# lmb-freiburg/understanding_flow_robustness

Hardware: AMD Instinct MI355X
Metric: attack-iters/s (higher is better)
Workload: dtype f32

## Files before the change

include/ufr_hip.h:

```cpp
#ifndef UFR_HIP_H_
#define UFR_HIP_H_

#include <stdint.h>

#ifdef __cplusplus
extern "C" {
#endif

#define UFR_ABI_VERSION 9

enum { UFR_F32 = 0, UFR_F64 = 1, UFR_F16 = 2 };
enum {
  UFR_OK = 0,
  UFR_EINVAL = -1,
  UFR_EUNSUPPORTED = -2,
  UFR_ELAUNCH = -3
};

typedef void* ufr_stream_t;

int ufr_abi_version(void);
const char* ufr_last_error(void);
int ufr_device_count(void);
const char* ufr_build_manifest(void);
// ... 337 lines not shown
                               void* c3a, long c3a_stride, void* c3b, long c3b_stride, float* c3_nchw, float* c3w_nchw,
                               const int* win, int B, int H, int W, int wh, int ww, int m2, int m3, ufr_stream_t stream);
int ufr_chunks_to_nchw(const void* planes, long plane_stride, const float* f32, int chunk0, const void* mask,
                       int mask_chunk0, float* out, int B, int C, int H, int W, float scale, float slope,
                       ufr_stream_t stream);
int ufr_nchw_cat_to_planes(const float* const* srcs, const int* channels, const int* dst_channel0, int nseg, void* planes,
                           long plane_stride, int chunk0, int chunks, int B, int H, int W, ufr_stream_t stream);
int ufr_chunks_to_nchw_cat(const float* g, int chunk0, int chunks, float* const* dsts, const int* channels, const int* src_channel0,
                           int nseg, const float* act0, float pos0, float neg0, int B, int H, int W, ufr_stream_t stream);
int ufr_grad_finalize(const float* g, int g_chunk0, const void* mask, int mask_chunk0, void* out, long out_plane_stride,
                      int out_chunk0, long M, int chunks, float slope, ufr_stream_t stream);

int ufr_conv1_direct(const float* frames_a, const float* frames_b, int Ba, int Bb, int H, int W, const double* mean,
                     const void* wimg, const float* bias, float slope, void* out_planes, long plane_stride, int out_chunk0,
                     ufr_stream_t stream);
int ufr_conv1_pack_planes(const float* frames_a, const float* frames_b, void* planes, long plane_stride, int Ba, int Bb, int H,
                          int W, const double* mean, ufr_stream_t stream);
int ufr_conv1_unpack_grad(const float* G, float* grad_frames, int N, int H, int W, ufr_stream_t stream);
int ufr_unshuffle_pack_planes(const float* x, void* planes, long plane_stride, int N, int C, int H, int W, ufr_stream_t stream);
int ufr_unshuffle_unpack_grad(const float* G, float* grad_x, int N, int C, int H, int W, ufr_stream_t stream);
int ufr_nchw_grad_to_planes(const float* grad, const float* act, void* planes, long plane_stride, int chunk0, int B, int C, int H,
                            int W, float slope, ufr_stream_t stream);
int ufr_window_gather_chunks(const float* src, float* dst, const int* win, int n_win, int N, int N_dst, int chunks, int Hs, int Ws,
                             int wh, int ww, int level_stride, int margin, ufr_stream_t stream);

int ufr_normalize_frames(const float* frames_a, const float* frames_b, float* out, int Ba, int Bb, int C, int H, int W,
                         const double* mean, ufr_stream_t stream);

int ufr_corr_forward_planes_window(const void* f1_planes, const void* f2_planes, long in_plane_stride, void* out_planes,
                                   long out_plane_stride, int out_chunk0, int B, int C, int H, int W, int patch,
                                   int dilation_patch, float scale, float slope, const int* win, int level_stride,
                                   int win_cells, ufr_stream_t stream);

int ufr_corr_backward_window_fused(const float* f1, const float* f2, const float* G, int g_chunk0, float g_scale,
                                   const float* G_redir, float* grad_window, int B, int C, int H, int W, int patch,
                                   int dilation_patch, const int* win, int level_stride, int wh, int ww, int margin,
                                   ufr_stream_t stream);

int ufr_corr_forward_planes(const void* f1_planes, const void* f2_planes, long in_plane_stride, void* out_planes,
                            long out_plane_stride, int out_chunk0, int B, int C, int H, int W, int patch,
                            int dilation_patch, float scale, float slope, ufr_stream_t stream);
int ufr_flow_head_planes_forward(const void* planes, long plane_stride, int chunk0, int chunks, const float* wpk, int w_chunks,
                                 const float* bias, float* out, int B, int H, int W, ufr_stream_t stream);
int ufr_flow_head_planes_forward_mfma(const void* planes, long plane_stride, int chunk0, int chunks, const void* wmf, int w_chunks,
                                      const float* bias, float* out, int B, int H, int W, ufr_stream_t stream);
int ufr_deconv_flow_tail_backward_mfma(const void* grad_planes, long plane_stride, int chunk0, int chunks, const void* wmf,
                                       int w_chunks, float* G, int g_chunks, int out_chunk, int B, int H, int W, ufr_stream_t stream);
int ufr_flow_head_planes_backward(const float* grad_y, const float* wpk, int w_chunks, float* G, int g_chunks, int chunk0, int chunks,
                                  int B, int H, int W, int accumulate, ufr_stream_t stream);
int ufr_flow_head_planes_backward_finalize(const float* grad_y, const float* wpk, int w_chunks, float* G, int g_chunks, int chunk0,
                                           int chunks, int B, int H, int W, int accumulate, const void* mask_planes, void* out_planes,
                                           long out_plane_stride, int fin_chunk0, int fin_chunks, float slope, ufr_stream_t stream);
#define UFR_PF_REGION_BAND 1
#define UFR_PF_REGION_WINDOW 2
int ufr_flow_head_planes_backward_regions(const float* grad_y, const float* wpk, int w_chunks, float* G, int g_chunks, int chunk0,
                                          int chunks, int B, int H, int W, int accumulate, int head_chunks, int region,
                                          const int* origin, int origin_stride, int origin_div, int reg_h, int reg_w, int margin,
                                          float* head_out, int head_out_images, const void* mask_planes, void* out_planes,
                                          long out_plane_stride, int fin_chunk0, int fin_chunks, float slope, ufr_stream_t stream);
int ufr_upfeat_planes_forward_mfma(const void* planes, long plane_stride, int chunk0, int chunks, const void* wmf, int w_chunks,
                                   const float* bias, float* out, int B, int H, int W, ufr_stream_t stream);
int ufr_upfeat_planes_backward(const float* grad_y, const float* wpk, int w_chunks, float* G, int g_chunks, int chunk0, int chunks,
                               int B, int H, int W, int accumulate, ufr_stream_t stream);
int ufr_flow_up_planes_forward(const float* x, const float* w, const float* bias, void* planes, long plane_stride,
                               int chunk, int B, int H, int W, ufr_stream_t stream);
int ufr_flow_up_planes_backward(const float* G, int chunk, const float* w, float* grad_x, int B, int H, int W,
// ... 38 lines not shown
```

understanding_flow_robustness_amd/_lib.py:

```python
from __future__ import annotations

import ctypes as C
import os

import torch

_HERE = os.path.dirname(os.path.abspath(__file__))
LIB_PATH = os.environ.get("UFR_HIP_LIB") or os.path.join(_HERE, "lib", "libufr_hip.so")
UFR_F32, UFR_F64, UFR_F16 = 0, 1, 2
ABI_VERSION = 9
_lib = None


class CorrParams(C.Structure):
    _fields_ = [(n, C.c_int) for n in (
        "kH", "kW", "patchH", "patchW", "padH", "padW", "dilationH", "dilationW",
        "dilation_patchH", "dilation_patchW", "dH", "dW")]


UFR_MAX_LEVELS = 8


class Pyramid(C.Structure):
    _fields_ = [("num_levels", C.c_int),
# ... 176 lines not shown
    "ufr_flow_head_planes_forward_mfma": [_vp, _l, _i, _i, _vp, _i, _vp, _vp, _i, _i, _i, _vp],
    "ufr_deconv_flow_tail_backward_mfma": [_vp, _l, _i, _i, _vp, _i, _vp, _i, _i, _i, _i, _i, _vp],
    "ufr_flow_head_planes_backward": [_vp, _vp, _i, _vp, _i, _i, _i, _i, _i, _i, _i, _vp],
    "ufr_flow_head_planes_backward_finalize": [_vp, _vp, _i, _vp, _i, _i, _i, _i, _i, _i, _i, _vp, _vp, _l, _i, _i, _f, _vp],
    "ufr_flow_head_planes_backward_regions": [_vp, _vp, _i, _vp, _i, _i, _i, _i, _i, _i, _i, _i, _i, _vp, _i, _i, _i, _i, _i, _vp, _i,
                                              _vp, _vp, _l, _i, _i, _f, _vp],
    "ufr_unshuffle_pack_planes": [_vp, _vp, _l, _i, _i, _i, _i, _vp],
    "ufr_unshuffle_unpack_grad": [_vp, _vp, _i, _i, _i, _i, _vp],
    "ufr_conv3x3s2_c3_planes": [_vp, _vp, _vp, _f, _vp, _l, _i, _i, _i, _i, _i, _vp],
    "ufr_conv3x3_c16_planes": [_vp, _l, _i, _vp, _vp, _f, _vp, _l, _i, _i, _i, _i, _vp],
    "ufr_cm_norm_stats": [_vp, _vp, _vp, _l, _i, _i, _f, _vp],
    "ufr_cm_norm_apply": [_vp, _vp, _vp, _l, _i, _vp, _l, _i, _l, _i, _i, _i, _i, _vp],
    "ufr_cm_norm_stats_apply": [_vp, _vp, _vp, _f, _vp, _l, _i, _vp, _l, _i, _l, _i, _i, _i, _i, _vp],
    "ufr_cm_norm_backward": [_vp, _vp, _vp, _i, _vp, _vp, _vp, _vp, _l, _i, _l, _i, _i, _i, _vp],
    "ufr_cm_masked_copy": [_vp, _vp, _l, _vp, _l, _vp],
    "ufr_raft_flow_patches": [_vp, _vp, _l, _i, _i, _i, _i, _vp],
    "ufr_raft_motion_finish_slabs": [_vp, _i, _i, _i, _vp, _f, _vp, _l, _vp, _l, _i, _vp, _i, _i, _i, _vp],
    "ufr_raft_motion_finish": [_vp, _l, _vp, _l, _i, _vp, _i, _i, _i, _vp],
    "ufr_raft_coords_step": [_vp, _vp, _vp, _vp, _vp, _l, _vp],
    "ufr_grad_finalize_consume": [_vp, _vp, _vp, _l, _l, _i, _f, _vp],
    "ufr_gru_gates_cm_forward": [_vp, _vp, _l, _i, _vp, _l, _i, _l, _i, _vp],
    "ufr_gru_gates_cm_forward_slabs": [_vp, _i, _i, _vp, _vp, _vp, _vp, _l, _i, _vp, _l, _i, _l, _i, _vp],
    "ufr_gru_blend_cm_forward_slabs": [_vp, _i, _i, _vp, _vp, _vp, _vp, _vp, _l, _i, _vp, _l, _i, _l, _i, _vp],
    "ufr_gru_blend_cm_forward": [_vp, _vp, _vp, _l, _i, _vp, _l, _i, _l, _i, _vp],
    "ufr_gru_blend_cm_backward": [_vp, _vp, _vp, _l, _i, _vp, _vp, _l, _i, _vp, _vp, _l, _i, _vp, _vp],
    "ufr_gru_gates_cm_backward": [_vp, _vp, _l, _i, _vp, _vp, _vp, _l, _i, _vp, _l, _i, _i, _vp, _vp],
    "ufr_altcorr_pyramid_forward": [_vp, _vp, _vp, _vp, _i, _i, _i, _i, _i, _f, _vp],
    "ufr_altcorr_pyramid_backward": [_vp, _vp, _vp, _vp, _vp, _vp, _i, _i, _i, _i, _i, _f, _i, _vp],
    "ufr_altcorr_pyramid_backward_cm": [_vp, _vp, _vp, _vp, _vp, _vp, _i, _i, _i, _i, _i, _f, _i, _vp],
    "ufr_upfeat_planes_forward_mfma": [_vp, _l, _i, _i, _vp, _i, _vp, _vp, _i, _i, _i, _vp],
    "ufr_upfeat_planes_backward": [_vp, _vp, _i, _vp, _i, _i, _i, _i, _i, _i, _i, _vp],
    "ufr_flow_up_planes_forward": [_vp, _vp, _vp, _vp, _l, _i, _i, _i, _i, _vp],
    "ufr_flow_up_planes_backward": [_vp, _i, _vp, _vp, _i, _i, _i, _i, _vp],
    "ufr_corr_forward_planes_window": [_vp, _vp, _l, _vp, _l, _i, _i, _i, _i, _i, _i, _i, _f, _f, _vp, _i, _i, _vp],
    "ufr_corr_forward_planes": [_vp, _vp, _l, _vp, _l, _i, _i, _i, _i, _i, _i, _i, _f, _f, _vp],
    "ufr_convex_upsample_forward": [_vp, _vp, _vp, _i, _i, _i, _vp],
    "ufr_convex_upsample_backward": [_vp, _vp, _vp, _vp, _vp, _vp, _i, _i, _i, _vp],
    "ufr_affine_resample_f64": [_vp, _vp, _i, _i, _i, _i, _i, _d, _d, _d, _d, _d, _d, _i, _vp],
    "ufr_patch_place": [_vp, _vp, _vp, _i, _i, _i, _vp, _vp, _vp, _i, _i, _i, _i, _vp],
    "ufr_patch_crop_f64": [_vp, _vp, _vp, _i, _i, _i, _i, _i, _i, _i, _vp],
    "ufr_resample_u8_horizontal": [_vp, _vp, _i, _i, _i, _i, _i, _vp, _vp, _i, _vp],
    "ufr_resample_u8_vertical": [_vp, _vp, _i, _i, _i, _i, _vp, _vp, _i, _vp],
    "ufr_u8_to_tensor": [_vp, _vp, _i, _i, _i, _i, _i, _i, _i, _f, _vp],
    "ufr_kitti_flow_decode": [_vp, _vp, _i, _i, _vp],
    "ufr_host_png_unfilter": [_vp, _vp, _i, _i, _i],
    "ufr_igemm_clock_probe": [_vp, _i],
    "ufr_altcorr_planes_prepare": [_vp, _vp, _l, _l, _i, _vp],
    "ufr_altcorr_planes_forward": [_vp, _l, C.POINTER(AltCorrPlaneLevels), _vp, _vp, _i, _i, _i, _i, _i, _f, _vp],
    "ufr_conv1_direct": [_vp, _vp, _i, _i, _i, _i, _vp, _vp, _vp, _f, _vp, _l, _i, _vp],
    "ufr_train_loss": [C.POINTER(TrainLossDesc), _vp],
    "ufr_grad_norm": [C.POINTER(AdamwSeg), _i, _f, _vp, _l, _vp, _vp],
    "ufr_adamw_step": [C.POINTER(AdamwSeg), _i, C.POINTER(AdamwHyper), _vp, _vp],
    "ufr_sweep_paste": [_vp, _vp, _vp, _vp, _vp, _vp, _vp, _vp, _i, _i, _i, _i, _i, _f, _f, C.POINTER(ConeChain), _i, _i, _vp, _vp, _vp],
    "ufr_sweep_metrics": [_vp, _vp, _vp, _vp, _vp, _i, _i, _i, _i, _i, _i, _i, _i, _vp, _l, _vp, _i, _i, _vp],
}
PLAIN = {"ufr_abi_version": (C.c_int, []), "ufr_last_error": (C.c_char_p, []),
         "ufr_device_count": (C.c_int, []), "ufr_build_manifest": (C.c_char_p, []),
         "ufr_igemm_variant_fallbacks": (C.c_int, []),
         "ufr_conv3x3_c2_workspace_floats": (C.c_long, [_i, _i, _i, _i]),
         "ufr_cm_norm_workspace_doubles": (C.c_long, [_l, _i, _i]),
         "ufr_resample2d_backward_workspace_bytes": (C.c_long, [_i, _i, _i]),
         "ufr_pwc_warp_backward_workspace_bytes": (C.c_long, [_i, _i, _i]),
         "ufr_altcorr_pyramid_workspace_bytes": (C.c_long, [_i, _i, _i, _i, _i, _i]),
         "ufr_train_loss_workspace_doubles": (C.c_long, [_i, _i, C.POINTER(C.c_int), C.POINTER(C.c_int)]),
         "ufr_grad_norm_partials": (C.c_long, [C.POINTER(AdamwSeg), _i]),
         "ufr_sweep_metrics_workspace_doubles": (C.c_long, [_i])}
# ... 263 lines not shown
```

understanding_flow_robustness_amd/csrc/correlation_planes.hip:

```cpp
#include "ufr_common.h"

namespace {

typedef __attribute__((ext_vector_type(8))) __bf16 bf16x8;
typedef __attribute__((ext_vector_type(4))) float f32x4;

__device__ constexpr int PROD_A[6] = {2, 0, 1, 1, 0, 0};
__device__ constexpr int PROD_B[6] = {0, 2, 1, 0, 1, 0};
__device__ __attribute__((aligned(64))) unsigned corr_zero_page[16];

__device__ __forceinline__ void glds16(const __bf16* src, __bf16* lds_wave_base) {
  __builtin_amdgcn_global_load_lds(src, lds_wave_base, 16, 0, 0);
}

__device__ __forceinline__ void split3(float v, __bf16& a, __bf16& b, __bf16& c) {
  a = (__bf16)v;
  const float r1 = v - (float)a;
  b = (__bf16)r1;
  c = (__bf16)(r1 - (float)b);
}

constexpr int P = 21, R = 10, KCH = 8;
constexpr int OT = 24;

// ... 136 lines not shown
        if (two) asm volatile("s_waitcnt vmcnt(6)" ::: "memory"); else asm volatile("s_waitcnt vmcnt(3)" ::: "memory");
      } else {
        asm volatile("s_waitcnt vmcnt(0)" ::: "memory");
      }
      asm volatile("s_waitcnt lgkmcnt(0)" ::: "memory");
      __builtin_amdgcn_s_barrier();
      cur = cur == 2 ? 0 : cur + 1;
      if (sl == KH - 1 && kh == 0) {
#pragma unroll
        for (int tt = 0; tt < 3; ++tt) {
          const f32x4 o = *reinterpret_cast<const f32x4*>(part + 4 * tt);
          acc[tt][0] += o[0]; acc[tt][1] += o[1]; acc[tt][2] += o[2]; acc[tt][3] += o[3];
        }
        write_row(dy, acc, false);
      }
    }
    t = tn;
  }
}

template <int NW>
int launch_corr_planes(const __bf16* a, const __bf16* b, long in_plane_stride, __bf16* o, long out_plane_stride, int out_chunk0,
                       int B, int H, int W, int ni, float scale, float slope, hipStream_t st, const int* win = nullptr,
                       int win_div = 1) {
  {
    hipError_t e = ufr::ensure_dynamic_lds(reinterpret_cast<const void*>(corr_fwd_planes_k2_kernel<NW>), corr_planes_k2_lds_bytes<NW>());
    if (e != hipSuccess) return ufr::fail(UFR_ELAUNCH, "correlation (planes): %s", hipGetErrorString(e));
  }
  corr_fwd_planes_k2_kernel<NW><<<dim3(win ? 1 : ufr::ceil_div(ni, 16 * NW), 2, B * H), 128 * NW, corr_planes_k2_lds_bytes<NW>(), st>>>(
      a, b, in_plane_stride, o, out_plane_stride, out_chunk0, B, H, W, scale, slope, win, win_div);
  return UFR_OK;
}

}

extern "C" int ufr_corr_forward_planes(const void* f1_planes, const void* f2_planes, long in_plane_stride, void* out_planes,
                                       long out_plane_stride, int out_chunk0, int B, int C, int H, int W, int patch,
                                       int dilation_patch, float scale, float slope, ufr_stream_t stream) {
  UFR_REQUIRE(f1_planes && f2_planes && out_planes, "correlation (planes): null pointer");
  UFR_REQUIRE(B > 0 && H > 0 && W > 0 && (long)B * H < 65536 && out_chunk0 >= 0, "correlation (planes): bad shape");
  if (C != 32 * KCH || patch != P || dilation_patch != 2)
    return ufr::fail(UFR_EUNSUPPORTED, "correlation (planes): built for FlowNetC's configuration (256 channels, patch 21, "
                                       "dilation_patch 2); got C=%d patch=%d dilation_patch=%d", C, patch, dilation_patch);
  const int ni = (W + 1) / 2;
  hipStream_t st = ufr::as_stream(stream);
  const __bf16* a = static_cast<const __bf16*>(f1_planes);
  const __bf16* b = static_cast<const __bf16*>(f2_planes);
  __bf16* o = static_cast<__bf16*>(out_planes);
  const int waves = ufr::ceil_div(ni, 16);
  int rc;
  if (waves <= 2) rc = launch_corr_planes<2>(a, b, in_plane_stride, o, out_plane_stride, out_chunk0, B, H, W, ni, scale, slope, st);
  else if (waves <= 4 || waves > 5 * 2)
    rc = launch_corr_planes<4>(a, b, in_plane_stride, o, out_plane_stride, out_chunk0, B, H, W, ni, scale, slope, st);
  else
    rc = launch_corr_planes<5>(a, b, in_plane_stride, o, out_plane_stride, out_chunk0, B, H, W, ni, scale, slope, st);
  if (rc != UFR_OK) return rc;
  return ufr::launched("corr_fwd_planes_kernel");
}

extern "C" int ufr_corr_forward_planes_window(const void* f1_planes, const void* f2_planes, long in_plane_stride, void* out_planes,
                                              long out_plane_stride, int out_chunk0, int B, int C, int H, int W, int patch,
                                              int dilation_patch, float scale, float slope, const int* win, int level_stride,
                                              int win_cells, ufr_stream_t stream) {
  UFR_REQUIRE(f1_planes && f2_planes && out_planes && win, "correlation (planes, window): null pointer");
  UFR_REQUIRE(B > 0 && H > 0 && W > 0 && (long)B * H < 65536 && out_chunk0 >= 0 && level_stride > 0 && win_cells > 0,
              "correlation (planes, window): bad shape");
  if (C != 32 * KCH || patch != P || dilation_patch != 2 || win_cells + 4 * R > 63)
    return ufr::fail(UFR_EUNSUPPORTED, "correlation (planes, window): 256 channels, patch 21, dilation_patch 2, windows of at most "
                                       "23 cells; got C=%d patch=%d dilation_patch=%d cells=%d", C, patch, dilation_patch, win_cells);
  int rc = launch_corr_planes<2>(static_cast<const __bf16*>(f1_planes), static_cast<const __bf16*>(f2_planes), in_plane_stride,
                                 static_cast<__bf16*>(out_planes), out_plane_stride, out_chunk0, B, H, W, (W + 1) / 2, scale, slope,
                                 ufr::as_stream(stream), win, level_stride);
  if (rc != UFR_OK) return rc;
  return ufr::launched("corr_fwd_planes_k2_kernel (window)");
}
```

understanding_flow_robustness_amd/flownetc_engine.py:

```python
from __future__ import annotations

import os

import torch
from ._lib import engine_cache as _engine_cache

from . import _lib as L
from . import igemm as ig

_HEADS = ((6, 1024), (5, 1026), (4, 770), (3, 386), (2, 194))


def _pack_flow_head(weight: torch.Tensor) -> torch.Tensor:
    cin = weight.shape[1]
    chunks = ig.pad32(cin) // 32
    w = torch.zeros(2, chunks * 32, 9, dtype=torch.float32, device=weight.device)
    w[:, :cin] = weight.detach().float().reshape(2, cin, 9)
    return w.view(2, chunks, 32, 9).permute(1, 3, 0, 2).contiguous()


def _pack_flow_head_mfma(weight: torch.Tensor) -> torch.Tensor:
    cin = weight.shape[1]
    chunks = ig.pad32(cin) // 32
    w = torch.zeros(chunks * 32, 32, dtype=torch.float32, device=weight.device)
# ... 13 lines not shown


class FlowNetCHeadEngine:
    def __init__(self, net, B: int, H: int, W: int, device):
        if H % 64 or W % 64:
            raise ValueError("FlowNetC head engine: frame sides must be multiples of 64")
        L.lib()
        self.net, self.B, self.H, self.W, self.dev = net, int(B), int(H), int(W), torch.device(device)
        g = {s: (H // s, W // s) for s in (4, 8, 16, 32, 64)}
        self.grid = g
        P = lambda s, chunks: ig.Planes(B, g[s][0], g[s][1], chunks, self.dev)
        G = lambda s, chunks: ig.GradSum(B, g[s][0], g[s][1], chunks, self.dev)
        self.siamese = hasattr(net, "conv_redir")
        self.c3a_p, self.c3b_p = (P(8, 8), P(8, 8)) if self.siamese else (None, None)
        self.in31, self.cat3, self.cat2 = P(8, 15 if self.siamese else 8), P(8, 13), P(4, 7)
        self.c4a, self.cat4 = P(16, 16), P(16, 25)
        self.c5a, self.cat5 = P(32, 16), P(32, 33)
        self.c6a, self.c6 = P(64, 32), P(64, 32)
        f32 = dict(dtype=torch.float32, device=self.dev)
        self.flow = {k: torch.zeros(B, 2, *g[2 ** k], **f32) for k in (6, 5, 4, 3, 2)}
        self.G_cat2, self.G_cat3, self.G_cat4, self.G_cat5 = G(4, 7), G(8, 13), G(16, 25), G(32, 33)
        self.G_c6, self.G_in31, self.G_c3a = G(64, 32), G(8, 15 if self.siamese else 8), G(8, 8)
        self.gz_cat2, self.gz_cat3, self.gz_cat4, self.gz_cat5 = P(4, 7), P(8, 13), P(16, 25), P(32, 33)
        self.gz_c6, self.gz_c6a, self.gz_c5a, self.gz_c4a = P(64, 32), P(64, 32), P(32, 16), P(16, 16)
        self.gz_in31 = P(8, 15) if self.siamese else None
        self.g_flow = {k: torch.zeros(B, 2, *g[2 ** k], **f32) for k in (6, 5, 4, 3)}
        self.g_corr = torch.zeros(B, 21, 21, *g[8], **f32)
        self.g_c2a = torch.zeros(B, 128, *g[4], **f32)
        self.g_c3a, self.g_c3a_redir, self.g_c3b = (torch.zeros(B, 256, *g[8], **f32) for _ in range(3))
        self.c3_nchw = torch.zeros(2 * B, 256, *g[8], **f32)
        self._prefix = None
        self.flow_out, self.flow_scale = self.flow[2], float(getattr(net, "div_flow", 20.0))
        self._wprefixes, self._wprefix = {}, None
        self._build_launches()

    def _conv(self, name):
        return getattr(self.net, name)[0]

    def _bias(self, conv):
        if conv.bias is None:
            return torch.zeros(conv.out_channels, dtype=torch.float32, device=self.dev)
        return conv.bias.detach().float().contiguous()

    def _stem_layers(self):
        from .plane_graph import stem_stages
        return [(name, block[0], lvl) for lvl, stage in enumerate(stem_stages(self.net), 1) for name, block in stage]

    def _build_launches(self):
        net, g, B = self.net, self.grid, self.B
        plans = []

        def plan(wi, x, in_chunk0, rows, out_hw, **kw):
            M = B * rows[0] * rows[1]
            pk = [len(t) * wi.KC for _, _, t in wi.phases]
            kw.setdefault("variant", self._variant_for(wi))
            bm, target = self._tile_rows_and_slots(wi, kw)
            S = ig.splitk_for(M, wi.Npad, max(pk), len(wi.phases), phase_ktiles=pk, bm=bm, target=target)
            kw["variant"], S = ig.tuned(wi, M, kw, kw["variant"], S, rows=rows)
            plans.append((wi, x, in_chunk0, rows, out_hw, S, kw))
            return len(plans) - 1

        self._pipe_variant = {"0": 2, "5": 5}.get(os.environ.get("UFR_IGEMM_PIPE", "6"), 6)

        fwd, bwd = {}, {}
        cw = lambda n, s, p: ig.conv_forward_weights(self._conv(n).weight, s, p)
        cb = lambda n, s, p: ig.conv_backward_weights(self._conv(n).weight, s, p)
# ... 133 lines not shown
        pk = P["packed"]
        L.check(L.lib().ufr_conv1_pack_planes(L.ptr(a), L.ptr(b.contiguous()) if b is not None else None, L.ptr(pk.t),
                                              pk.plane_stride, int(a.shape[0]), nb, int(a.shape[2]), int(a.shape[3]),
                                              L.ptr(mean), L.stream()), "conv1 pack")
        P["conv1"]()

    def prefix_full(self, frames_a: torch.Tensor, frames_b: torch.Tensor):
        if self._prefix is None:
            self._build_prefix()
        B = self.B

        def chain(h, frames, out):
            P = self._prefix[h]
            self._conv1(P, frames, None)
            for _, launch, _ in P["layers"]:
                launch()
            (self.c3a_p if h == "a" else self.c3b_p).to_nchw(256, 0, out=out)
        chain("a", frames_a, self.c3_nchw[:B])
        chain("b", frames_b, self.c3_nchw[B:])
        self._c3a, self._c3b = self.c3_nchw[:B], self.c3_nchw[B:]

    def load_prefix_features(self, c2_all: torch.Tensor, c3_all: torch.Tensor):
        B = self.B
        self.cat2.load_nchw(c2_all[:B].contiguous(), 0)
        self.c3_nchw.copy_(c3_all[:2 * B])
        self._c3a, self._c3b = self.c3_nchw[:B], self.c3_nchw[B:]
        self.c3a_p.load_nchw(self._c3a, 0)
        self.c3b_p.load_nchw(self._c3b, 0)

    def scatter_window_features(self, c2_w: torch.Tensor, c3_w: torch.Tensor, win: torch.Tensor, wh: int, ww: int, m2: int, m3: int):
        lib, B, st = L.lib(), self.B, L.stream()
        h4, w4 = self.grid[4]
        h8, w8 = self.grid[8]
        L.check(lib.ufr_window_scatter_planes(L.ptr(c2_w), L.ptr(self.cat2.t), self.cat2.plane_stride, 0, L.ptr(win), B, B, 128,
                                              h4, w4, wh // 4, ww // 4, 4, m2, st), "window -> planes (conv2)")
        for k, dst in ((0, self.c3a_p), (1, self.c3b_p)):
            L.check(lib.ufr_window_scatter_planes(L.ptr(c3_w[k * B:]), L.ptr(dst.t), dst.plane_stride, 0, L.ptr(win), B, B, 256,
                                                  h8, w8, wh // 8, ww // 8, 8, m3, st), "window -> planes (conv3)")
        L.check(lib.ufr_window_scatter(L.ptr(c3_w), L.ptr(self.c3_nchw), L.ptr(win), B, 2 * B, 256, h8, w8, wh // 8, ww // 8, 8,
                                       m3, st), "window -> nchw (conv3)")

    def _build_window_prefix(self, wh: int, ww: int):
        B2, dev = 2 * self.B, self.dev
        f32 = dict(dtype=torch.float32, device=dev)
        h2, w2, h4, w4, h8, w8 = wh // 2, ww // 2, wh // 4, ww // 4, wh // 8, ww // 8
        layers = self._stem_layers()
        n = len(layers)
        tap2 = max(i for i, (_, _, lvl) in enumerate(layers) if lvl == 2)
        acts = [ig.Planes(B2, wh >> lvl, ww >> lvl, ig.pad32(conv.out_channels) // 32, dev) for _, conv, lvl in layers]
        gz = [ig.Planes(B2, wh >> lvl, ww >> lvl, ig.pad32(conv.out_channels) // 32, dev) for _, conv, lvl in layers]
        G_p = ig.GradSum(B2, h2 + 3, w2 + 2, 1, dev)
        G_gw2 = ig.GradSum(B2, h4, w4, 4, dev)
        grid = lambda i: (wh >> layers[i][2], ww >> layers[i][2])
        plans, names = [], []
        for i in range(1, n):
            name, conv, _ = layers[i]
            plans.append((ig.conv_forward_weights(conv.weight, conv.stride[0], conv.padding[0]), acts[i - 1], grid(i), grid(i),
                          dict(out_planes=acts[i], bias=self._bias(conv), variant=4)))
            names.append(name)
        for i in range(n - 1, 0, -1):
            name, conv, _ = layers[i]
            kw = dict(add=G_gw2, mask=acts[i - 1], out_planes=gz[i - 1]) if i - 1 == tap2 else dict(out_planes=gz[i - 1], mask=acts[i - 1])
            plans.append((ig.conv_backward_weights(conv.weight, conv.stride[0], conv.padding[0]), gz[i], grid(i), grid(i - 1), kw))
            names.append(name + "_bwd")
        plans.append((ig.conv1_packed_backward_weights(layers[0][1].weight), gz[0], (h2 + 3, w2 + 2), (h2 + 3, w2 + 2),
                      dict(out_f32=G_p)))
# ... 8 lines not shown
        ws = torch.empty(need, **f32)
        launches = [ig.make_launch(wi, x, 0, rows, out_hw, splitk=S, ws=ws if S > 1 else None, **kw)
                    for (wi, x, rows, out_hw, kw), S in zip(plans, sized)]
        chain = [(name, launch, p[0]) for name, launch, p in zip(names, launches, plans)]
        P = dict(hw=(wh, ww), c1=acts[0], c2=acts[tap2], c3=acts[-1], gz_c3=gz[-1], gz_c2=gz[tap2], G_gw2=G_gw2, ws=ws,
                 acts=acts, gz=gz, fwd=chain[:n - 1], bwd=chain[n - 1:],
                 G_p=G_p, gxw=torch.zeros(B2, 3, wh, ww, **f32),
                 c2_nchw=torch.zeros(B2, 128, h4, w4, **f32), c3_nchw=torch.zeros(B2, 256, h8, w8, **f32))
        P.update({name: launch for name, launch, _ in chain})
        P.update({name + "_wi": wi for name, _, wi in chain})
        P.update(self._conv1_launch(B2, wh, ww, acts[0]))
        self._wprefixes[(wh, ww)] = P
        self._bound_wprefixes()
        return P

    MAX_WINDOW_PREFIXES = 4

    def _bound_wprefixes(self):
        while len(self._wprefixes) > self.MAX_WINDOW_PREFIXES:
            del self._wprefixes[next(iter(self._wprefixes))]

    def window_prefix(self, wh: int, ww: int) -> dict:
        P = self._wprefixes.pop((int(wh), int(ww)), None)
        if P is None:
            P = self._build_window_prefix(int(wh), int(ww))
        else:
            self._wprefixes[(int(wh), int(ww))] = P
        self._wprefix = P
        return P

    def window_prefix_forward(self, xw: torch.Tensor, win: torch.Tensor, m2: int, m3: int, c2_nchw: bool = True):
        wh, ww = int(xw.shape[2]), int(xw.shape[3])
        P = self.window_prefix(wh, ww)
        self._conv1(P, xw.detach(), None)
        for _, launch, _ in P["fwd"]:
            launch()
        c2, c3, H, W = P["c2"], P["c3"], self.H, self.W
        L.check(L.lib().ufr_window_features_planes(
            L.ptr(c2.t), c2.plane_stride, L.ptr(c3.t), c3.plane_stride, L.ptr(self.cat2.t), self.cat2.plane_stride,
            L.ptr(self.c3a_p.t), self.c3a_p.plane_stride, L.ptr(self.c3b_p.t), self.c3b_p.plane_stride, L.ptr(self.c3_nchw),
            L.ptr(P["c3_nchw"]), L.ptr(win), self.B, H, W, wh, ww, int(m2), int(m3), L.stream()), "window features -> planes")
        if c2_nchw:
            c2.to_nchw(128, 0, out=P["c2_nchw"])

    def window_gather_conv2_gradient(self, win: torch.Tensor, m2: int):
        P = self._wprefix
        wh, ww = P["hw"]
        h4, w4 = self.grid[4]
        L.check(L.lib().ufr_window_gather_chunks(L.ptr(self.G_cat2.t), L.ptr(P["G_gw2"].t), L.ptr(win), self.B, self.B, 2 * self.B, 4,
                                                 h4, w4, wh // 4, ww // 4, 4, int(m2), L.stream()), "window gather (chunks)")

    def window_prefix_backward(self, gw3: torch.Tensor, gw2: torch.Tensor | None = None, unpack: bool = True) -> torch.Tensor:
        P, B = self._wprefix, self.B
        wh, ww = P["hw"]
        if gw2 is not None:
            full = torch.zeros(2 * B, 128, wh // 4, ww // 4, dtype=torch.float32, device=self.dev)
            full[:B] = gw2
            P["G_gw2"].t.copy_(full.view(2 * B, 4, 32, wh // 4, ww // 4).permute(1, 0, 3, 4, 2).reshape(4, -1, 32))
        gz = P["gz_c3"]
        L.check(L.lib().ufr_nchw_grad_to_planes(L.ptr(gw3), L.ptr(P["c3_nchw"]), L.ptr(gz.t), gz.plane_stride, 0, 2 * B, 256, wh // 8,
                                                ww // 8, ig.LEAKY, L.stream()), "window gradient -> planes")
        for _, launch, _ in P["bwd"]:
            launch()
        if not unpack:
            return P["G_p"].t
        L.check(L.lib().ufr_conv1_unpack_grad(L.ptr(P["G_p"].t), L.ptr(P["gxw"]), 2 * B, wh, ww, L.stream()), "conv1 unpack")
# ... 175 lines not shown
                                                   L.ptr(dst.t), dst.plane_stride, chunk, self.B, f.shape[2], f.shape[3],
                                                   L.stream()), "upsampled_flow forward")

    def _deconv_tail(self, k):
        src, chunk0, chunks, Gd, out_chunk, (h, w) = self.tail_args[k]
        L.check(L.lib().ufr_deconv_flow_tail_backward_mfma(L.ptr(src.t), src.plane_stride, chunk0, chunks, L.ptr(self.tail_w[k]),
                                                           self.tail_w[k].shape[0], L.ptr(Gd.t), Gd.chunks, out_chunk, self.B, h, w, L.stream()),
                "deconv data gradient, flow channels")

    def _up_backward(self, k):
        G, chunk = self.up_G[k]
        f = self.g_flow[k]
        L.check(L.lib().ufr_flow_up_planes_backward(L.ptr(G.t), chunk, L.ptr(self.up_w[k]), L.ptr(f), self.B, f.shape[2],
                                                    f.shape[3], 0, L.stream()), "upsampled_flow backward")

    def _finalize(self, Gs, mask, out, chunk0, chunks):
        L.check(L.lib().ufr_grad_finalize(L.ptr(Gs.t), chunk0, L.ptr(mask.t), chunk0, L.ptr(out.t), out.plane_stride, chunk0,
                                          Gs.M, chunks, ig.LEAKY, L.stream()), "gradient finalize")

    def _forward_trunk(self, c2: torch.Tensor, c3: torch.Tensor) -> torch.Tensor:
        L.require_hip(c2, "c2")
        L.require_hip(c3, "c3")
        self.cat2.load_nchw(c2, 0)
        self.in31.load_nchw(c3, 0)
        for name in ("conv3_1", "conv4", "conv4_1", "conv5", "conv5_1", "conv6", "conv6_1"):
            self.fwd[name]()
        self._pf_forward(6)
        for k in (5, 4, 3, 2):
            self._up_forward(k + 1)
            self.fwd[f"deconv{k}"]()
            self._pf_forward(k)
        return self.flow[2]

    def forward_cached(self, band=None) -> torch.Tensor:
        return self.forward(None, self._c3a, self._c3b, band)

    def forward(self, c2a: torch.Tensor | None, c3a: torch.Tensor, c3b: torch.Tensor, band=None) -> torch.Tensor:
        if not self.siamese:
            return self._forward_trunk(c2a, c3a)
        for t, name in ((c3a, "c3a"), (c3b, "c3b")):
            L.require_hip(t, name)
        self._c3a, self._c3b = c3a, c3b
        inc = False
        if band is not None:
            self.attach_band(band)
            inc = bool(band.width and band.incremental and band.inc_layers)
        if c2a is not None:
            L.require_hip(c2a, "c2a")
            self.cat2.load_nchw(c2a, 0)
            self.c3a_p.load_nchw(c3a, 0)
            self.c3b_p.load_nchw(c3b, 0)
        if inc and band.cone_win is not None and band.cone_hw[1] // 8 <= 23:
            L.check(L.lib().ufr_corr_forward_planes_window(L.ptr(self.c3a_p.t), L.ptr(self.c3b_p.t), self.c3a_p.plane_stride,
                                                           L.ptr(self.in31.t), self.in31.plane_stride, 1, self.B, 256, *self.grid[8],
                                                           21, 2, 1.0 / 256.0, ig.LEAKY, L.ptr(band.cone_win), 8,
                                                           band.cone_hw[1] // 8, L.stream()), "correlation forward (planes, window)")
        else:
            L.check(L.lib().ufr_corr_forward_planes(L.ptr(self.c3a_p.t), L.ptr(self.c3b_p.t), self.c3a_p.plane_stride,
                                                    L.ptr(self.in31.t), self.in31.plane_stride, 1, self.B, 256, *self.grid[8], 21, 2,
                                                    1.0 / 256.0, ig.LEAKY, L.stream()), "correlation forward (planes)")
        for name in ("conv_redir", "conv3_1", "conv4", "conv4_1"):
            (self.fwd_band if inc else self.fwd)[name]()
        for name in ("conv5", "conv5_1", "conv6", "conv6_1"):
            self.fwd[name]()
        self._pf_forward(6)
        for k in (5, 4, 3, 2):
            self._up_forward(k + 1)
            self.fwd[f"deconv{k}"]()
            self._pf_forward(k)
        return self.flow[2]

    def backward(self, g_flow2: torch.Tensor, band=None, fused_window: bool = True, skip_unread: bool = True):
        L.require_hip(g_flow2, "g_flow2")
        B = self.B
        banded = band is not None and bool(band.width)
        if band is not None:
            self.attach_band(band)
        gz = {2: (self.G_cat2, self.cat2, self.gz_cat2, 4, 2), 3: (self.G_cat3, self.cat3, self.gz_cat3, 8, 4),
              4: (self.G_cat4, self.cat4, self.gz_cat4, 16, 8), 5: (self.G_cat5, self.cat5, self.gz_cat5, 16, 16)}
        fuse = os.environ.get("UFR_FUSE_FINALIZE", "1") != "0"
        fin = lambda k: (gz[k][1], gz[k][2], gz[k][3], gz[k][4]) if fuse else None
        eng_window = bool(fused_window and band is not None and getattr(band, "eng_window", False)
                          and getattr(self, "_wprefix", None) is not None)
        skip = bool(skip_unread and banded and fused_window and self.siamese)
        if skip and eng_window:
            P = self._wprefix
            wh, ww = P["hw"]
            self._pf_backward(2, g_flow2, accumulate=False, finalize=fin(2),
                              region=(4, L.UFR_PF_REGION_WINDOW, band.cone_win, 8, 4, wh // 4, ww // 4, band.g2_margin, P["G_gw2"]))
# ... 110 lines not shown
```

understanding_flow_robustness_amd/patch_attack.py:

```python
from __future__ import annotations

import ctypes as C
import os
from argparse import Namespace

import numpy as np
import torch
from ._lib import engine_cache as _engine_cache

from . import _lib as L
from .flownets.utils_model import predict_flow

LOSS_THRESHOLD = 0.1
CLAMP_BOUND = 2.0


def _pixel_range(flownet: str):
    return (0.0, 1.0) if any(k in flownet for k in ("FlowNetC", "FlowNetS", "FlowNet2", "RAFT", "PWC")) else (-1.0, 1.0)


class ShardedExchange:

    def __init__(self, group=None):
        import torch.distributed as dist
        self.dist, self.group = dist, group
        self.world = dist.get_world_size(group) if dist.is_initialized() else 1
        self.rank = dist.get_rank(group) if dist.is_initialized() else 0

    def __call__(self, packed: torch.Tensor) -> torch.Tensor:
        if self.world > 1:
            self.dist.all_reduce(packed, op=self.dist.ReduceOp.SUM, group=self.group)
        return packed

    def gather(self, rows_local: torch.Tensor, rows_all: torch.Tensor) -> torch.Tensor:
        if self.world > 1:
            self.dist.all_gather_into_tensor(rows_all, rows_local, group=self.group)
        return rows_all


class PatchAttackStep:

    def __init__(self, flow_net, args, batch, height, width, device="cuda:0", shared_patch=True,
                 exchange: ShardedExchange | None = None, use_graph=True, warmup=3, use_cone=None, patch_hw=None,
                 sum_groups=1, skip_unread=True):
        L.lib()
        self.net, self.args = flow_net, args
        self.skip_unread = bool(skip_unread)
        self.B, self.H, self.W = batch, height, width
        self.dev = torch.device(device)
        self.shared = shared_patch
        self.exchange = exchange
        self.world = exchange.world if exchange is not None else 1
        if self.world > 1 and not shared_patch:
            raise ValueError("per-sample patches need no exchange; shard them as independent replicas")
        self.placed = patch_hw is not None
        if shared_patch and batch * self.world > 1 and not self.placed:
            raise ValueError("one patch behind several pairs is defined in patch coordinates: pass patch_hw=(ph, pw) "
                             "and load() a [1,3,ph,pw] patch / mask with per-pair origins (SURVEY.md 8e)")
        if self.placed and not shared_patch:
            raise ValueError("patch_hw: per-sample patches stay canvas-sized like the reference's")
        self.groups = int(sum_groups)
        if self.groups < 1 or batch % self.groups or (self.groups > 1 and not self.placed):
            raise ValueError("sum_groups must divide the pairs of a patch-coordinate step")
        self.lo, self.hi = _pixel_range(args.flownet)
        self.kind = 1 if getattr(args, "l2", False) else 0
        self.alpha = float(getattr(args, "alpha", 0.0))
        self.step = 0.5 * float(args.lr)
        self.CHW = 3 * height * width
        f32 = dict(dtype=torch.float32, device=self.dev)
        pb = 1 if shared_patch else batch
        self.tgt = torch.zeros(batch, 3, height, width, **f32)
        self.ref = torch.zeros_like(self.tgt)
        self._mask_canvas = None if self.placed else torch.zeros_like(self.tgt)
        self._mask_stale = self.placed
        if self.placed:
            ph, pw = (int(v) for v in patch_hw)
            if not (0 < ph <= height and 0 < pw <= width):
                raise ValueError("patch_hw does not fit the frame")
            self.ph, self.pw, self.n_p = ph, pw, 3 * ph * pw
            self.patch = torch.zeros(1, 3, ph, pw, **f32)
# ... 168 lines not shown
            self.band.win[:, 1] = start.clamp(0, self.W - self.band.width)
            if self.band.corr_width:
                from .band_conv import corr_band_origin
                self.band.win[:, 2] = corr_band_origin(self.win[:, 1], self.band.corr_width, self.W)
        self._cone_prefix(prefix_features)

    def _cone_prefix(self, prefix_features=None):
        if self.eng is not None:
            if prefix_features is not None:
                self.eng.load_prefix_features(*prefix_features)
            else:
                self.eng.prefix_full(self.adv_tgt.detach(), self.adv_ref.detach())
            return
        feats = prefix_features if prefix_features is not None else \
            self.net.encode(torch.cat((self.adv_tgt.detach(), self.adv_ref.detach()), 0))
        for (ls, m, n, full, _), f in zip(self.taps, feats):
            if f.shape[0] < n or f.shape[1:] != full.shape[1:]:
                raise ValueError("prefix_features do not match this step's frames")
            full.detach().copy_(f[:n])

    def _forward_cone(self):
        lib, B, H, W = L.lib(), self.B, self.H, self.W
        wh, ww = self.win_hw
        L.check(lib.ufr_window_gather_pair(L.ptr(self.adv_tgt), L.ptr(self.adv_ref), L.ptr(self.xw), L.ptr(self.win),
                                           L.ptr(self.loss_local), B, 3, H, W, wh, ww, L.stream()), "window gather (pair)")
        if self.eng is not None:
            self._feats_w = None
            if self.eng_kind == "pwc":
                self.eng.window_prefix_forward(self.xw, self.win, self.taps[0][1])
                self.eng.forward_cached()
            else:
                (_, m2, _, _, _), (_, m3, _, _, _) = self.taps
                self.eng.window_prefix_forward(self.xw, self.win, m2, m3, c2_nchw=False)
                self.eng.forward_cached(self.band)
            if self._fused_loss:
                return None
            return torch.nn.functional.interpolate(self.eng.flow_out * self.eng.flow_scale, scale_factor=4, mode="bilinear",
                                                   align_corners=False)
        self._feats_w = [f[:n] for f, (_, _, n, _, _) in zip(self.net.encode(self.xw), self.taps)]
        for f, (ls, m, n, full, _) in zip(self._feats_w, self.taps):
            self._win_copy(lib.ufr_window_scatter, f, full, n, f.shape[1], H // ls, W // ls, ls, m)
        full = [t[3] for t in self.taps]
        extra = {"band": self.band} if self.band is not None else {}
        return self.net.head(*full[:-1], full[-1][:B], full[-1][B:], **extra)

    def _backward_cone(self, flow):
        lib, B, H, W = L.lib(), self.B, self.H, self.W
        self._packed_grad = False
        if self.eng is not None:
            if flow is None:
                g_flow2 = self.g_flow2
            else:
                (g_flow2,) = torch.autograd.grad(flow, (self.eng.flow_out,), self.g_flow)
            if self.eng_kind == "pwc":
                ls, m, n, _, gw = self.taps[0]
                g_f2 = self.eng.backward(g_flow2.contiguous())
                self._win_copy(lib.ufr_window_gather, g_f2, gw, n, g_f2.shape[1], H // ls, W // ls, ls, m)
                gxw = self.eng.window_prefix_backward(gw)
            else:
                (ls2, m2, _, _, gw2), (ls3, m3, _, _, gw3) = self.taps
                if self.band is not None:
                    self.band.g3_window, self.band.g3_margin = gw3, m3
                    self.band.eng_window, self.band.g2_margin = True, m2
                g2a, g3a, g3b = self.eng.backward(g_flow2.contiguous(), self.band, skip_unread=self.skip_unread)
                if g2a is not None:
                    self._win_copy(lib.ufr_window_gather, g2a, gw2, B, 128, H // ls2, W // ls2, ls2, m2)
                if g3a is not None:
# ... 372 lines not shown
```

Before: 1489.

## Recompute FlowNetC correlation only for rows touched by the changed window

```diff
diff --git a/include/ufr_hip.h b/include/ufr_hip.h
--- a/include/ufr_hip.h
+++ b/include/ufr_hip.h
@@ -393,6 +393,11 @@
                                    int dilation_patch, float scale, float slope, const int* win, int level_stride,
                                    int win_cells, ufr_stream_t stream);
 
+int ufr_corr_forward_planes_changed(const void* f1_planes, const void* f2_planes, long in_plane_stride, void* out_planes,
+                                    long out_plane_stride, int out_chunk0, int B, int C, int H, int W, int patch,
+                                    int dilation_patch, float scale, float slope, const int* win, int level_stride,
+                                    int win_cells_h, int win_cells_w, int margin, ufr_stream_t stream);
+
 int ufr_corr_backward_window_fused(const float* f1, const float* f2, const float* G, int g_chunk0, float g_scale,
                                    const float* G_redir, float* grad_window, int B, int C, int H, int W, int patch,
                                    int dilation_patch, const int* win, int level_stride, int wh, int ww, int margin,
diff --git a/understanding_flow_robustness_amd/_lib.py b/understanding_flow_robustness_amd/_lib.py
--- a/understanding_flow_robustness_amd/_lib.py
+++ b/understanding_flow_robustness_amd/_lib.py
@@ -232,6 +232,7 @@
     "ufr_upfeat_planes_backward": [_vp, _vp, _i, _vp, _i, _i, _i, _i, _i, _i, _i, _vp],
     "ufr_flow_up_planes_forward": [_vp, _vp, _vp, _vp, _l, _i, _i, _i, _i, _vp],
     "ufr_flow_up_planes_backward": [_vp, _i, _vp, _vp, _i, _i, _i, _i, _vp],
+    "ufr_corr_forward_planes_changed": [_vp, _vp, _l, _vp, _l, _i, _i, _i, _i, _i, _i, _i, _f, _f, _vp, _i, _i, _i, _i, _vp],
     "ufr_corr_forward_planes_window": [_vp, _vp, _l, _vp, _l, _i, _i, _i, _i, _i, _i, _i, _f, _f, _vp, _i, _i, _vp],
     "ufr_corr_forward_planes": [_vp, _vp, _l, _vp, _l, _i, _i, _i, _i, _i, _i, _i, _f, _f, _vp],
     "ufr_convex_upsample_forward": [_vp, _vp, _vp, _i, _i, _i, _vp],
diff --git a/understanding_flow_robustness_amd/csrc/correlation_planes.hip b/understanding_flow_robustness_amd/csrc/correlation_planes.hip
--- a/understanding_flow_robustness_amd/csrc/correlation_planes.hip
+++ b/understanding_flow_robustness_amd/csrc/correlation_planes.hip
@@ -192,6 +192,139 @@
   return UFR_OK;
 }
 
+constexpr int CH_WAVES = 4;
+constexpr int CH_MAX_CELLS = 23;
+
+__device__ __forceinline__ bf16x8 load_fragment(const __bf16* src, int perm) {
+  typedef __attribute__((ext_vector_type(4))) int i32x4;
+  i32x4 v = *reinterpret_cast<const i32x4*>(src);
+#pragma unroll
+  for (int k = 0; k < 4; ++k) v[k] = __builtin_amdgcn_ds_bpermute(perm, v[k]);
+  return __builtin_bit_cast(bf16x8, v);
+}
+
+template <bool CASE_B>
+__device__ __forceinline__ void corr_changed_rows(const __bf16* __restrict__ f1, const __bf16* __restrict__ f2, long in_plane_stride,
+                                                  __bf16* __restrict__ out, long out_plane_stride, int out_chunk0, long M, int W,
+                                                  float scale, float slope, long rowS, long rowD, long row1, int rx0, int rx1, int dy,
+                                                  float* otile, int lane) {
+  const __bf16* zero = reinterpret_cast<const __bf16*>(corr_zero_page);
+  const int fr = lane & 15, g = lane >> 4;
+  const int lc = lane >> 2, perm = ((fr << 2) | g) << 2;
+  const __bf16* baseS = (CASE_B ? f2 : f1) + rowS * 32 + (lane & 3) * 8;
+  const __bf16* baseD = (CASE_B ? f1 : f2) + rowD * 32 + (lane & 3) * 8;
+  int i_lo[2], n[2];
+  bool s_ok[2], d_ok[2][2];
+  const __bf16 *sp[2], *dp[2][2];
+#pragma unroll
+  for (int par = 0; par < 2; ++par) {
+    i_lo[par] = (rx0 - par + 1) >> 1;
+    n[par] = ((rx1 - par + 1) >> 1) - i_lo[par];
+    s_ok[par] = lc < n[par];
+    sp[par] = baseS + (long)(2 * (i_lo[par] + lc) + par) * 32;
+#pragma unroll
+    for (int t = 0; t < 2; ++t) {
+      const int u = i_lo[par] - R + 16 * t + lc, xu = 2 * u + par;
+      d_ok[par][t] = u >= 0 && xu < W;
+      dp[par][t] = baseD + (long)xu * 32;
+    }
+  }
+  f32x4 acc[2][2][2];
+#pragma unroll
+  for (int h = 0; h < 2; ++h)
+#pragma unroll
+    for (int par = 0; par < 2; ++par)
+#pragma unroll
+      for (int t = 0; t < 2; ++t) acc[h][par][t] = f32x4{0.f, 0.f, 0.f, 0.f};
+#pragma unroll
+  for (int c = 0; c < KCH; ++c) {
+    const long off = (long)c * M * 32;
+    bf16x8 fs[2][3], fd[2][2][3];
+#pragma unroll
+    for (int p = 0; p < 3; ++p)
+#pragma unroll
+      for (int par = 0; par < 2; ++par)
+        fs[par][p] = load_fragment(s_ok[par] ? sp[par] + p * in_plane_stride + off : zero, perm);
+#pragma unroll
+    for (int p = 0; p < 3; ++p)
+#pragma unroll
+      for (int t = 0; t < 2; ++t)
+#pragma unroll
+        for (int par = 0; par < 2; ++par)
+          fd[par][t][p] = load_fragment(d_ok[par][t] ? dp[par][t] + p * in_plane_stride + off : zero, perm);
+#pragma unroll
+    for (int par = 0; par < 2; ++par)
+#pragma unroll
+      for (int q = 0; q < 6; ++q)
+#pragma unroll
+        for (int t = 0; t < 2; ++t) {
+          f32x4& a = acc[c / (KCH / 2)][par][t];
+          a = CASE_B ? __builtin_amdgcn_mfma_f32_16x16x32_bf16(fd[par][t][PROD_A[q]], fs[par][PROD_B[q]], a, 0, 0, 0)
+                     : __builtin_amdgcn_mfma_f32_16x16x32_bf16(fs[par][PROD_A[q]], fd[par][t][PROD_B[q]], a, 0, 0, 0);
+        }
+  }
+  constexpr int ROWS = 32;
+#pragma unroll
+  for (int par = 0; par < 2; ++par) {
+#pragma unroll
+    for (int t = 0; t < 2; ++t)
+#pragma unroll
+      for (int rg = 0; rg < 4; ++rg) {
+        const float v = acc[0][par][t][rg] + acc[1][par][t][rg];
+        const int m = g * 4 + rg;
+        const int il = CASE_B ? 16 * t + m : m;
+        const int dx = CASE_B ? fr - il + 2 * R : 16 * t + fr - m;
+        if (dx >= 0 && dx < P && (!CASE_B || fr < n[par])) otile[il * OT + dx] = v;
+      }
+    const int np = n[par], cnt = (CASE_B ? ROWS : P) * np;
+    for (int e = lane; e < cnt; e += 64) {
+      const int il = CASE_B ? e / np : e / P;
+      const int dx = CASE_B ? e - il * np - il + 2 * R : e - il * P;
+      const int i = CASE_B ? i_lo[par] - R + il : i_lo[par] + il, x = 2 * i + par;
+      if (!CASE_B || (dx >= 0 && dx < P && i >= 0 && x < W)) {
+        float v = otile[il * OT + dx] * scale;
+        v = v > 0.f ? v : v * slope;
+        __bf16 p0, p1, p2;
+        split3(v, p0, p1, p2);
+        const int d = dy * P + dx;
+        __bf16* o = out + ((long)(out_chunk0 + (d >> 5)) * M + row1 + x) * 32 + (d & 31);
+        o[0] = p0;
+        o[out_plane_stride] = p1;
+        o[2 * out_plane_stride] = p2;
+      }
+    }
+  }
+}
+
+__global__ __launch_bounds__(64 * CH_WAVES, 3) void corr_fwd_planes_changed_kernel(
+    const __bf16* __restrict__ f1, const __bf16* __restrict__ f2, long in_plane_stride, __bf16* __restrict__ out, long out_plane_stride,
+    int out_chunk0, int B, int H, int W, float scale, float slope, const int* __restrict__ win, int level_stride, int wh, int ww,
+    int margin) {
+  __shared__ float tiles[CH_WAVES][32 * OT];
+  const int lane = threadIdx.x & 63;
+  const int wave = __builtin_amdgcn_readfirstlane(threadIdx.x >> 6);
+  const int groups = ((wh + 1) / 2 + CH_WAVES - 1) / CH_WAVES;
+  int item = blockIdx.x;
+  const int k = item % groups; item /= groups;
+  const int yd = item % H; item /= H;
+  const int case_b = item & 1, b = item >> 1;
+  if (b >= B) return;
+  const int wy0 = min(max(win[b * 8 + 0] / level_stride, 0), H - wh), wx0 = min(max(win[b * 8 + 1] / level_stride, 0), W - ww);
+  const int ry0 = wy0 + (wy0 > 0 ? margin : 0), ry1 = wy0 + wh - (wy0 + wh < H ? margin : 0);
+  const int rx0 = wx0 + (wx0 > 0 ? margin : 0), rx1 = wx0 + ww - (wx0 + ww < W ? margin : 0);
+  const int ys = ry0 + ((ry0 ^ yd) & 1) + 2 * (k * CH_WAVES + wave);
+  const int dy = (case_b ? ys - yd : yd - ys) / 2 + R;
+  if (ys >= ry1 || dy < 0 || dy >= P || rx1 <= rx0) return;
+  const long M = (long)B * H * W;
+  const long rowS = ((long)b * H + ys) * W, rowD = ((long)b * H + yd) * W;
+  if (case_b)
+    corr_changed_rows<true>(f1, f2, in_plane_stride, out, out_plane_stride, out_chunk0, M, W, scale, slope, rowS, rowD, rowD, rx0, rx1, dy,
+                            tiles[wave], lane);
+  else
+    corr_changed_rows<false>(f1, f2, in_plane_stride, out, out_plane_stride, out_chunk0, M, W, scale, slope, rowS, rowD, rowS, rx0, rx1, dy,
+                             tiles[wave], lane);
+}
+
 }
 
 extern "C" int ufr_corr_forward_planes(const void* f1_planes, const void* f2_planes, long in_plane_stride, void* out_planes,
@@ -234,3 +367,23 @@
   if (rc != UFR_OK) return rc;
   return ufr::launched("corr_fwd_planes_k2_kernel (window)");
 }
+
+extern "C" int ufr_corr_forward_planes_changed(const void* f1_planes, const void* f2_planes, long in_plane_stride, void* out_planes,
+                                               long out_plane_stride, int out_chunk0, int B, int C, int H, int W, int patch,
+                                               int dilation_patch, float scale, float slope, const int* win, int level_stride,
+                                               int win_cells_h, int win_cells_w, int margin, ufr_stream_t stream) {
+  UFR_REQUIRE(f1_planes && f2_planes && out_planes && win, "correlation (planes, changed): null pointer");
+  UFR_REQUIRE(B > 0 && H > 0 && W > 0 && (long)B * H < 65536 && out_chunk0 >= 0 && level_stride > 0 && win_cells_h > 0 &&
+                  win_cells_w > 0 && margin >= 0, "correlation (planes, changed): bad shape");
+  if (C != 32 * KCH || patch != P || dilation_patch != 2 || win_cells_w > CH_MAX_CELLS)
+    return ufr::fail(UFR_EUNSUPPORTED, "correlation (planes, changed): 256 channels, patch 21, dilation_patch 2, windows of at most "
+                                       "%d cells across; got C=%d patch=%d dilation_patch=%d cells=%d", CH_MAX_CELLS, C, patch,
+                     dilation_patch, win_cells_w);
+  UFR_REQUIRE(win_cells_h <= H && win_cells_w <= W && 2 * margin <= win_cells_h && 2 * margin <= win_cells_w,
+              "correlation (planes, changed): window %dx%d (margin %d) in a frame of %dx%d cells", win_cells_h, win_cells_w, margin, H, W);
+  const int groups = ufr::ceil_div((win_cells_h + 1) / 2, CH_WAVES);
+  corr_fwd_planes_changed_kernel<<<B * 2 * H * groups, 64 * CH_WAVES, 0, ufr::as_stream(stream)>>>(
+      static_cast<const __bf16*>(f1_planes), static_cast<const __bf16*>(f2_planes), in_plane_stride, static_cast<__bf16*>(out_planes),
+      out_plane_stride, out_chunk0, B, H, W, scale, slope, win, level_stride, win_cells_h, win_cells_w, margin);
+  return ufr::launched("corr_fwd_planes_changed_kernel");
+}
diff --git a/understanding_flow_robustness_amd/flownetc_engine.py b/understanding_flow_robustness_amd/flownetc_engine.py
--- a/understanding_flow_robustness_amd/flownetc_engine.py
+++ b/understanding_flow_robustness_amd/flownetc_engine.py
@@ -69,6 +69,7 @@
         self._prefix = None
         self.flow_out, self.flow_scale = self.flow[2], float(getattr(net, "div_flow", 20.0))
         self._wprefixes, self._wprefix = {}, None
+        self._win_m3 = 0
         self._build_launches()
 
     def _conv(self, name):
@@ -268,6 +269,7 @@
         lib, B, st = L.lib(), self.B, L.stream()
         h4, w4 = self.grid[4]
         h8, w8 = self.grid[8]
+        self._win_m3 = int(m3)
         L.check(lib.ufr_window_scatter_planes(L.ptr(c2_w), L.ptr(self.cat2.t), self.cat2.plane_stride, 0, L.ptr(win), B, B, 128,
                                               h4, w4, wh // 4, ww // 4, 4, m2, st), "window -> planes (conv2)")
         for k, dst in ((0, self.c3a_p), (1, self.c3b_p)):
@@ -342,6 +344,7 @@
     def window_prefix_forward(self, xw: torch.Tensor, win: torch.Tensor, m2: int, m3: int, c2_nchw: bool = True):
         wh, ww = int(xw.shape[2]), int(xw.shape[3])
         P = self.window_prefix(wh, ww)
+        self._win_m3 = int(m3)
         self._conv1(P, xw.detach(), None)
         for _, launch, _ in P["fwd"]:
             launch()
@@ -583,10 +586,11 @@
             self._pf_forward(k)
         return self.flow[2]
 
-    def forward_cached(self, band=None) -> torch.Tensor:
-        return self.forward(None, self._c3a, self._c3b, band)
-
-    def forward(self, c2a: torch.Tensor | None, c3a: torch.Tensor, c3b: torch.Tensor, band=None) -> torch.Tensor:
+    def forward_cached(self, band=None, corr_changed: bool = True) -> torch.Tensor:
+        return self.forward(None, self._c3a, self._c3b, band, corr_changed=corr_changed)
+
+    def forward(self, c2a: torch.Tensor | None, c3a: torch.Tensor, c3b: torch.Tensor, band=None,
+                corr_changed: bool = True) -> torch.Tensor:
         if not self.siamese:
             return self._forward_trunk(c2a, c3a)
         for t, name in ((c3a, "c3a"), (c3b, "c3b")):
@@ -602,10 +606,17 @@
             self.c3a_p.load_nchw(c3a, 0)
             self.c3b_p.load_nchw(c3b, 0)
         if inc and band.cone_win is not None and band.cone_hw[1] // 8 <= 23:
-            L.check(L.lib().ufr_corr_forward_planes_window(L.ptr(self.c3a_p.t), L.ptr(self.c3b_p.t), self.c3a_p.plane_stride,
-                                                           L.ptr(self.in31.t), self.in31.plane_stride, 1, self.B, 256, *self.grid[8],
-                                                           21, 2, 1.0 / 256.0, ig.LEAKY, L.ptr(band.cone_win), 8,
-                                                           band.cone_hw[1] // 8, L.stream()), "correlation forward (planes, window)")
+            if corr_changed:
+                L.check(L.lib().ufr_corr_forward_planes_changed(L.ptr(self.c3a_p.t), L.ptr(self.c3b_p.t), self.c3a_p.plane_stride,
+                                                                L.ptr(self.in31.t), self.in31.plane_stride, 1, self.B, 256, *self.grid[8],
+                                                                21, 2, 1.0 / 256.0, ig.LEAKY, L.ptr(band.cone_win), 8,
+                                                                band.cone_hw[0] // 8, band.cone_hw[1] // 8, self._win_m3, L.stream()),
+                        "correlation forward (planes, changed)")
+            else:
+                L.check(L.lib().ufr_corr_forward_planes_window(L.ptr(self.c3a_p.t), L.ptr(self.c3b_p.t), self.c3a_p.plane_stride,
+                                                               L.ptr(self.in31.t), self.in31.plane_stride, 1, self.B, 256, *self.grid[8],
+                                                               21, 2, 1.0 / 256.0, ig.LEAKY, L.ptr(band.cone_win), 8,
+                                                               band.cone_hw[1] // 8, L.stream()), "correlation forward (planes, window)")
         else:
             L.check(L.lib().ufr_corr_forward_planes(L.ptr(self.c3a_p.t), L.ptr(self.c3b_p.t), self.c3a_p.plane_stride,
                                                     L.ptr(self.in31.t), self.in31.plane_stride, 1, self.B, 256, *self.grid[8], 21, 2,
diff --git a/understanding_flow_robustness_amd/patch_attack.py b/understanding_flow_robustness_amd/patch_attack.py
--- a/understanding_flow_robustness_amd/patch_attack.py
+++ b/understanding_flow_robustness_amd/patch_attack.py
@@ -42,10 +42,11 @@
 
     def __init__(self, flow_net, args, batch, height, width, device="cuda:0", shared_patch=True,
                  exchange: ShardedExchange | None = None, use_graph=True, warmup=3, use_cone=None, patch_hw=None,
-                 sum_groups=1, skip_unread=True):
+                 sum_groups=1, skip_unread=True, corr_changed=True):
         L.lib()
         self.net, self.args = flow_net, args
         self.skip_unread = bool(skip_unread)
+        self.corr_changed = bool(corr_changed)
         self.B, self.H, self.W = batch, height, width
         self.dev = torch.device(device)
         self.shared = shared_patch
@@ -280,7 +281,7 @@
             else:
                 (_, m2, _, _, _), (_, m3, _, _, _) = self.taps
                 self.eng.window_prefix_forward(self.xw, self.win, m2, m3, c2_nchw=False)
-                self.eng.forward_cached(self.band)
+                self.eng.forward_cached(self.band, corr_changed=self.corr_changed)
             if self._fused_loss:
                 return None
             return torch.nn.functional.interpolate(self.eng.flow_out * self.eng.flow_scale, scale_factor=4, mode="bilinear",
```

After: 1505, median of 6. 1.1% higher.
